# VikParuchuri/surya

Measured on AMD Instinct MI355X. Metric: text-lines/sec recognised (whole node), higher is better.
Workload: dtype bf16; 1 GPU; RecognitionPredictor device loop, 256 ragged 64x{128..512} crops/GPU, batch 256, max_tokens=48, REC-FULL synthetic weights (conditioned recipe, seed 0), tiles resident in HBM; parallelism=1 GPU, weights=conditioned

## Files before the change

surya_amd/csrc/common.h:

```cpp
#pragma once
#include <hip/hip_runtime.h>
#include <cstdlib>
#include <stdint.h>
#include <stdio.h>
#include <type_traits>

#include "../../include/surya_amd.h"

namespace sa {

typedef unsigned short bf16_t;
typedef __attribute__((ext_vector_type(4))) float f32x4;
typedef __attribute__((ext_vector_type(16))) float f32x16;
typedef __attribute__((ext_vector_type(8))) __bf16 bf16x8;
typedef unsigned int u32x4 __attribute__((ext_vector_type(4)));


#define SA_HIP(expr)                                                                                   \
    do {                                                                                               \
        hipError_t _e = (expr);                                                                        \
        if (_e != hipSuccess) {                                                                        \
            fprintf(stderr, "[surya_amd] %s:%d %s -> %s\n", __FILE__, __LINE__, #expr, hipGetErrorString(_e)); \
            return (int)_e;                                                                            \
        }                                                                                              \
// ... 228 lines not shown
    int graph = 0;
    int split_target = 256;
    int split_min_kt = 4;
    int split_max = 8;
    int bigtile = 3;
    int bigtile_any = 0;
    int big_m_split = -1;
    int big_m_gateup = -1;
    int mx_big_m_split = -1;
    int mx_big_m_gateup = -1;
    int gateup_ring = 2;
    int dring = 1;
    int dring_min_kt = 0;
    int conv_persist = 3;
    int dwconv_pipe = 2;
    int conv_lean = 1;
    int bigtile_ratio_pct = 0;
    int bigtile_min_k = 0;
    int glds = 2;
    int dattn = 4;
    int rnorm = 2;
    int ghead = 2;
    int fuse_embed = 1;
    int kvprefetch = 0;
    int lmhead = 1;
    int dattn_db = 0;
    int lay_ln = 1;
    int det_head_blk = 1;
    int det_fuse = 1023;
    int det_up4 = 1;
    int fmb_chunk = 64;
    int persist = 1;
    int ocrerr_cls_only = 1;
};
inline Tuning& tuning() { static Tuning t; return t; }
inline int& tuning_epoch() { static int e = 0; return e; }

inline void poison_arena(void* p, size_t bytes) {
    static const bool on = [] { const char* e = getenv("SURYA_AMD_POISON"); return e && e[0] == '1'; }();
    if (on) { (void)hipMemset(p, 0xFF, bytes); (void)hipDeviceSynchronize(); }
}

struct AttrOnce {
    size_t granted[64] = {};
    template <typename F> void ensure(F kern, size_t lds) {
        int dev = 0;
        (void)hipGetDevice(&dev);
        size_t& g = granted[dev & 63];
        if (lds > g || g == 0) {
            (void)hipFuncSetAttribute(reinterpret_cast<const void*>(kern), hipFuncAttributeMaxDynamicSharedMemorySize, (int)lds);
            g = lds > g ? lds : g;
            if (g == 0) g = 1;
        }
    }
};

constexpr int SA_ALT_NONE = 0x7fffffff;
__device__ __forceinline__ bool alt_after(float v, int c, float pv, int pc) { return (v < pv) | ((v == pv) & (c > pc)); }
__device__ __forceinline__ bool alt_before(float v, int c, float bv, int bc) { return (v > bv) | ((v == bv) & (c < bc)); }
__device__ __forceinline__ float2 alt_next(const float2* cand, int n, float pv, int pc) {
    float cb = -INFINITY;
    int ci = SA_ALT_NONE;
    for (int k = 0; k < n; ++k) {
        const float v = cand[k].x;
        const int cc = __float_as_int(cand[k].y);
        const bool take = (v > -INFINITY) & alt_after(v, cc, pv, pc) & alt_before(v, cc, cb, ci);
// ... 11 lines not shown
```

surya_amd/csrc/gemm.h:

```cpp
#pragma once
#include <algorithm>
#include <cstdlib>
#include <type_traits>

#include "common.h"
#include "fastdiv.h"

namespace sa {

enum GemmEpi { EPI_BIAS = 0, EPI_RESIDUAL = 1, EPI_GELU = 2, EPI_SWIGLU = 3, EPI_HARDSWISH = 4, EPI_RELU = 5, EPI_ARGMAX = 6, EPI_ROPE = 7,
               EPI_GEGLU = 8 ,
               EPI_ARGMAX_MASK = 9 ,
               EPI_TOPK = 10 ,
               EPI_FORCED = 11  };
constexpr bool epi_is_argmax(int epi) { return epi == EPI_ARGMAX || epi == EPI_ARGMAX_MASK || epi == EPI_TOPK || epi == EPI_FORCED; }
constexpr bool epi_is_masked(int epi) { return epi == EPI_ARGMAX_MASK || epi == EPI_TOPK; }

struct TokenMask {
    const uint32_t* table = nullptr;
    const int* slot_mask = nullptr;
    const int* row_slot = nullptr;
    int words = 0;
    __device__ __forceinline__ int id_of(int m, int M) const {
        const int gm = min(m, M - 1);
// ... 1578 lines not shown
    const bool prof = pf.enabled && pf.n < GemmProfiler::POOL;
    if (prof) (void)hipEventRecord(pf.ev[2 * pf.n], s);
    hipLaunchKernelGGL(kern, dim3(grid), dim3(512), lds, s, aa);
    if (prof) {
        (void)hipEventRecord(pf.ev[2 * pf.n + 1], s);
        pf.cfg_of[pf.n] = CONV ? 3 : gemm_cfg_id(BM, BN);
        pf.flops_of[pf.n] = CONV ? 2.0 * a.M * a.N * a.cTaps * a.cCin : 2.0 * a.M * a.N * a.K;
        const double outn = (EPI == EPI_SWIGLU || EPI == EPI_GEGLU) ? a.N / 2 : a.N;
        const double xelems = CONV ? (double)a.M / std::max(1, a.cHo * a.cWo) * a.cH * a.cW * a.cCin : (double)a.M * a.K;
        pf.bytes_of[pf.n] = (xelems + (double)a.N * a.K) * sizeof(TI) + (double)a.M * outn * sizeof(TO) +
                            (EPI == EPI_RESIDUAL ? (double)a.M * a.N * sizeof(TO) : 0.0);
        pf.slab_of[pf.n] = 0.0;
        ++pf.n;
    }
    return (int)hipGetLastError();
}

}
#include "gemm_ring.h"
namespace sa {

static inline bool gemm_misaligned(const void* p, size_t bytes) { return (reinterpret_cast<uintptr_t>(p) & (bytes - 1)) != 0; }
template <typename TI, typename TO>
static inline bool gemm_operands_ok(const GemmArgs<TI, TO>& a, bool with_r) {
    constexpr long CI = 16 / (long)sizeof(TI), CO = 16 / (long)sizeof(TO);
    if (a.K <= 0 || a.ldx % CI != 0 || a.ldw % CI != 0 || a.ldc % CO != 0) return false;
    if (gemm_misaligned(a.X, 16) || gemm_misaligned(a.W, 16) || gemm_misaligned(a.C, 16) || gemm_misaligned(a.part, 16)) return false;
    if (gemm_misaligned(a.bias, 4 * sizeof(TI))) return false;
    if (with_r && (a.ldr % CO != 0 || gemm_misaligned(a.R, 16))) return false;
    return true;
}

template <typename TI, typename TO, int EPI>
static inline int launch_gemm(const GemmArgs<TI, TO>& a, hipStream_t s) {
    if (a.M <= 0 || a.N <= 0) return SA_OK;
    if (!gemm_operands_ok(a, EPI == EPI_RESIDUAL)) return SA_ERR_SHAPE;
    if constexpr (EPI == EPI_ROPE) {
        if (!a.rope || gemm_misaligned(a.rope, 16) || a.rope_D <= 0 || a.rope_D % 4 != 0 || a.rope_cols < 4 || a.rope_cols % 4 != 0) return SA_ERR_SHAPE;
    }
    {
        const int n_out = (EPI == EPI_SWIGLU || EPI == EPI_GEGLU) ? a.N / 2 : a.N;
        if (a.K % Ty<TI>::KE != 0 || a.N % 4 != 0 || n_out % (16 / (int)sizeof(TO)) != 0 || a.ldc % (16 / (int)sizeof(TO)) != 0)
            return SA_ERR_SHAPE;
    }
    if constexpr (EPI == EPI_ARGMAX_MASK) {
        if (!a.tmask.table || !a.tmask.slot_mask || a.tmask.words != cdiv(a.N, 32)) return SA_ERR_ARG;
    }
    if constexpr (EPI == EPI_TOPK) {
        if (!a.alt || (a.tmask.table && (!a.tmask.slot_mask || a.tmask.words != cdiv(a.N, 32)))) return SA_ERR_ARG;
    }
    if constexpr (EPI == EPI_FORCED) {
        if (!a.forced.table || !a.forced.flogit || a.forced.stride <= 0) return SA_ERR_ARG;
    }
    if (a.M <= 256) {
        if constexpr (epi_is_argmax(EPI)) {
            if (a.N >= 64 * 512 && tuning().lmhead && (a.K / Ty<TI>::KE) % 2 == 0 && a.N % 4 == 0) {
                if constexpr (sizeof(TI) == 2)
                    if (tuning().lmhead == 2) return launch_gemm_cfg<TI, TO, 256, 320, 4, 2, EPI, false, 2, false, 2>(a, s);
                return launch_gemm_cfg<TI, TO, 256, 320, 4, 2, EPI, false, 2>(a, s);
            }
            if (a.N >= 64 * 512) return launch_gemm_cfg<TI, TO, 128, 128, 2, 2, EPI, false, 2>(a, s);
            return launch_gemm_cfg<TI, TO, 64, 64, 2, 2, EPI, false, 2>(a, s);
        }
        if (a.M > 128) {
            if (a.N >= 64 * 512) return launch_gemm_cfg<TI, TO, 128, 128, 2, 2, EPI, false, 2>(a, s);
            if constexpr (EPI == EPI_SWIGLU && sizeof(TI) == 2 && sizeof(TO) == 2) {
                const int rc = launch_gateup_ring(a, s);
// ... 17 lines not shown
            GemmArgs<TI, TO> g = a;
            g.mgroup = 1;
            int rc;
            if constexpr (sizeof(TI) == 2) {
                if (tuning().lmhead == 2) { rc = launch_gemm_cfg<TI, TO, 256, 320, 4, 2, EPI, false, 2, false, 2>(g, s); a.bn_used = g.bn_used; return rc; }
            }
            rc = launch_gemm_cfg<TI, TO, 256, 320, 4, 2, EPI, false, 2>(g, s);
            a.bn_used = g.bn_used;
            return rc;
        }
    }
    if constexpr (EPI == EPI_SWIGLU && sizeof(TI) == 2 && sizeof(TO) == 2) {
        const int mode = tuning().big_m_gateup;
        const int rb = cdiv(a.M, 256), t256 = rb * cdiv(a.N, 256);
        const int pick = mode >= 0 ? mode : ((rb >= 4 && t256 >= 160 && t256 < 256) ? 2 : 0);
        if (pick && (a.K / Ty<TI>::KE) % 2 == 0 && a.K / Ty<TI>::KE >= 4 && a.N % 8 == 0) {
            if (pick == 1) return launch_gemm_persist<TI, TO, EPI>(a, s);
            return launch_gemm_cfg<TI, TO, 256, 256, 4, 2, EPI, false, 8>(a, s);
        }
    }
    if (a.N <= 64 && a.M >= 128 * 256) return launch_gemm_cfg<TI, TO, 128, 64, 4, 1, EPI>(a, s);
    const long big = (long)cdiv(a.M, 128) * cdiv(a.N, 128);
    const int glds = tuning().glds;
    if constexpr (sizeof(TO) == 2) {
        const int bigtile = tuning().bigtile;
        const long t256 = (long)cdiv(a.M, 256) * cdiv(a.N, 256);
        const double ratio256 = tuning().bigtile_ratio_pct > 0 ? tuning().bigtile_ratio_pct / 100.0
                                                                : ((bigtile == 3 && sizeof(TI) == 2) ? 1.4 : 1.17);
        const double cost256 = (double)cdivl(t256, 256) * 256 * 4 / ratio256, cost128 = (double)cdivl(big, 512) * 512;
        if (bigtile && a.K >= tuning().bigtile_min_k && ((t256 >= 256 && cost256 <= cost128) || tuning().bigtile_any)) {
            if constexpr (!epi_is_argmax(EPI)) {
                const int nk = a.K / Ty<TI>::KE;
                if constexpr (sizeof(TI) == 2)
                    if (tuning().persist && nk >= 4 && nk % 2 == 0 && a.N % 8 == 0) return launch_gemm_persist<TI, TO, EPI>(a, s);
            }
            if constexpr (sizeof(TI) == 2 && !epi_is_argmax(EPI)) {
                if (bigtile == 2 && (a.K / Ty<TI>::KE) % 2 == 0) return launch_gemm_cfg<TI, TO, 256, 256, 2, 2, EPI, false, 2>(a, s);
                if (bigtile == 3 && (a.K / Ty<TI>::KE) % 2 == 0) return launch_gemm_cfg<TI, TO, 256, 256, 4, 2, EPI, false, 8>(a, s);
            }
            return launch_gemm_cfg<TI, TO, 256, 256, 4, 2, EPI, false, 2>(a, s);
        }
    }
    if (big >= 256) {
        if (glds == 2) return launch_gemm_cfg<TI, TO, 128, 128, 2, 2, EPI, false, 2>(a, s);
        if (glds == 3) return launch_gemm_cfg<TI, TO, 128, 128, 2, 2, EPI, false, 3>(a, s);
        return launch_gemm_cfg<TI, TO, 128, 128, 2, 2, EPI>(a, s);
    }
    return launch_gemm_cfg<TI, TO, 64, 64, 2, 2, EPI>(a, s);
}

static inline int pick_splitk(int tiles_n, int nk) {
    const Tuning& t = tuning();
    const int tiles = tiles_n * 4;
    int s = (t.split_target + tiles / 2) / tiles;
    s = std::min(s, nk / std::max(1, t.split_min_kt));
    return std::max(1, std::min(s, std::min(t.split_max, 8)));
}

template <typename TI>
static inline int launch_gemm_splitk(GemmArgs<TI, TI>& a, hipStream_t s) {
    if (a.M <= 0 || a.N <= 0) return SA_OK;
    if (a.K % Ty<TI>::KE != 0 || a.N % 4 != 0 || !a.part) return SA_ERR_SHAPE;
    if (!gemm_operands_ok(a, false)) return SA_ERR_SHAPE;
    const int nk = a.K / Ty<TI>::KE;
    a.splitk = pick_splitk(cdiv(a.N, 64), nk);
    if constexpr (sizeof(TI) == 2) {
        const int mode = tuning().big_m_split;
// ... 14 lines not shown
```

surya_amd/csrc/kernels.h:

```cpp
#pragma once
#include "common.h"

#ifndef SA_DBG_VARIANT
#define SA_DBG_VARIANT 0
#endif

namespace sa {

template <typename T>
__global__ void convert_tiles_kernel(const float* __restrict__ in, T* __restrict__ out, const int* __restrict__ src_row,
                                     int P, int kin, int kout) {
    const int row = blockIdx.x;
    const float* src = in + (long)src_row[row] * kin;
    T* dst = out + (long)row * kout;
    for (int c = threadIdx.x * 4; c < kout; c += blockDim.x * 4) {
        float v[4];
#pragma unroll
        for (int r = 0; r < 4; ++r) v[r] = (c + r < kin) ? src[c + r] : 0.f;
        store4(dst + c, v[0], v[1], v[2], v[3]);
    }
}

template <typename T>
__global__ __launch_bounds__(256) void rmsnorm_kernel(const T* __restrict__ x, long ldx, const T* __restrict__ w,
// ... 118 lines not shown
#pragma unroll
            for (int jj = 0; jj < 16; ++jj) {
                const int j = jb + jj;
                if (j < nk) {
                    const float pj = __expf(s[jj] - mnew);
                    lrun += pj;
                    const T* vr = vs + j * D + sl * DS;
#pragma unroll
                    for (int i = 0; i < DS; i += 4) {
                        float t4[4];
                        load4(vr + i, t4);
                        acc[i] += pj * t4[0]; acc[i + 1] += pj * t4[1]; acc[i + 2] += pj * t4[2]; acc[i + 3] += pj * t4[3];
                    }
                }
            }
        }
        __syncthreads();
    }
    if (valid) {
        const float inv = 1.0f / lrun;
        T* op = out + sg.o_off[seg] + (long)qi * o_row + (long)head * o_head + sl * DS;
#pragma unroll
        for (int i = 0; i < DS; i += 4) store4(op + i, acc[i] * inv, acc[i + 1] * inv, acc[i + 2] * inv, acc[i + 3] * inv);
    }
}

template <typename T>
__global__ void scatter_rows_kernel(const T* __restrict__ src, const int* __restrict__ dst_row, T* __restrict__ dst, int H) {
    const int r = blockIdx.x;
    const T* s = src + (long)r * H;
    T* d = dst + (long)dst_row[r] * H;
    for (int c = threadIdx.x * Ty<T>::V16; c < H; c += blockDim.x * Ty<T>::V16)
        *reinterpret_cast<uint4*>(d + c) = *reinterpret_cast<const uint4*>(s + c);
}

template <typename T>
__global__ void scatter_image_kernel(const T* __restrict__ merged, const T* __restrict__ hemb, const T* __restrict__ wemb,
                                     const int* __restrict__ dst_row, const int* __restrict__ hidx, const int* __restrict__ widx,
                                     T* __restrict__ embeds, int H) {
    const int r = blockIdx.x;
    const T* src = merged + (long)r * H;
    const T* he = hemb + (long)hidx[r] * H;
    const T* we = wemb + (long)widx[r] * H;
    T* dst = embeds + (long)dst_row[r] * H;
    for (int c = threadIdx.x * 4; c < H; c += blockDim.x * 4) {
        float a[4], b[4], d[4];
        load4(src + c, a); load4(he + c, b); load4(we + c, d);
        store4(dst + c, a[0] + Ty<T>::rnd(b[0] + d[0]), a[1] + Ty<T>::rnd(b[1] + d[1]), a[2] + Ty<T>::rnd(b[2] + d[2]),
               a[3] + Ty<T>::rnd(b[3] + d[3]));
    }
}

template <typename T>
__global__ void embed_tokens_kernel(const T* __restrict__ table, const int* __restrict__ ids, T* __restrict__ x, int H) {
    const int t = blockIdx.x;
    const int id = ids[t];
    if (id < 0) return;
    const uint4* src = reinterpret_cast<const uint4*>(table + (long)id * H);
    uint4* dst = reinterpret_cast<uint4*>(x + (long)t * H);
    for (int c = threadIdx.x; c < H / Ty<T>::V16; c += blockDim.x) dst[c] = src[c];
}

template <typename T>
__global__ void rope_table_kernel(const float* __restrict__ inv_freq, float2* __restrict__ table, int Tmax, int half) {
    const int idx = blockIdx.x * blockDim.x + threadIdx.x;
    if (idx >= Tmax * half) return;
// ... 512 lines not shown
    hipLaunchKernelGGL(rmsnorm_kernel<T>, dim3(cdiv(rows, 4)), dim3(256), 0, s, x, ldx, w, y, ldy, src_row, rows, C, eps);
    return (int)hipGetLastError();
}

template <typename T>
int launch_convert_tiles(const float* in, T* out, const int* src_row, int P, int kin, int kout, hipStream_t s) {
    if (P <= 0) return SA_OK;
    if (kout % 4 || kin > kout) return SA_ERR_SHAPE;
    hipLaunchKernelGGL(convert_tiles_kernel<T>, dim3(P), dim3(64), 0, s, in, out, src_row, P, kin, kout);
    return (int)hipGetLastError();
}
inline int launch_rope_vision_table(const int* pos_hw, const float* inv_freq, float2* tab, int P, int D, hipStream_t s) {
    if (P <= 0) return SA_OK;
    if (D <= 0 || D % 4) return SA_ERR_SHAPE;
    hipLaunchKernelGGL(rope_vision_table_kernel, dim3((unsigned)cdivl((long)P * (D / 2), 256)), dim3(256), 0, s, pos_hw, inv_freq, tab, P, D);
    return (int)hipGetLastError();
}
template <typename T>
int launch_scatter_image(const T* merged, const T* hemb, const T* wemb, const int* dst_row, const int* hidx, const int* widx, T* embeds, int rows,
                         int H, hipStream_t s) {
    if (rows <= 0) return SA_OK;
    if (H % 4) return SA_ERR_SHAPE;
    hipLaunchKernelGGL(scatter_image_kernel<T>, dim3(rows), dim3(128), 0, s, merged, hemb, wemb, dst_row, hidx, widx, embeds, H);
    return (int)hipGetLastError();
}
template <typename T>
int launch_scatter_rows(const T* src, const int* dst_row, T* dst, int rows, int H, hipStream_t s) {
    if (rows <= 0) return SA_OK;
    if (H % Ty<T>::V16) return SA_ERR_SHAPE;
    hipLaunchKernelGGL(scatter_rows_kernel<T>, dim3((unsigned)rows), dim3(128), 0, s, src, dst_row, dst, H);
    return (int)hipGetLastError();
}
template <typename T>
int launch_embed_tokens(const T* table, const int* ids, T* x, int rows, int H, hipStream_t s) {
    if (rows <= 0) return SA_OK;
    if (H % Ty<T>::V16) return SA_ERR_SHAPE;
    hipLaunchKernelGGL(embed_tokens_kernel<T>, dim3(rows), dim3(128), 0, s, table, ids, x, H);
    return (int)hipGetLastError();
}
template <typename T>
int launch_rope_table(const float* inv_freq, float2* table, int Tmax, int half, hipStream_t s) {
    if (Tmax <= 0 || half <= 0 || (long)Tmax * half > 0x7fffffffL) return SA_ERR_SHAPE;
    hipLaunchKernelGGL(rope_table_kernel<T>, dim3(cdiv(Tmax * half, 256)), dim3(256), 0, s, inv_freq, table, Tmax, half);
    return (int)hipGetLastError();
}
template <typename T>
int launch_rope_kv_append(T* qkv, const int* tok_slot, const int* tok_pos, const float2* rope_cs, T* kc, T* vc, int M, int nq, int nkv, int D,
                          int Tmax, hipStream_t s) {
    if (M <= 0) return SA_OK;
    if (D <= 0 || D % 2 || nq <= 0 || nkv <= 0) return SA_ERR_SHAPE;
    hipLaunchKernelGGL(rope_kv_append_kernel<T>, dim3(M), dim3(256), 0, s, qkv, tok_slot, tok_pos, rope_cs, kc, vc, nq, nkv, D, Tmax);
    return (int)hipGetLastError();
}

template <typename T>
int launch_reduce_norm(const float* part, int S, int M, T* x, const T* w, T* y, int H, float eps, uint8_t* y8, uint8_t* sy, int srows,
                       const KvPrefetch& pf, hipStream_t s) {
    const int threads = cdiv(H / 4, 64) * 64;
    if (threads > 1024 || H % 4) return SA_ERR_UNSUPPORTED;
    const int grid = pf.base ? 2 * M : M;
#define SA_RNORM(SL) hipLaunchKernelGGL((splitk_residual_norm_kernel<T, SL>), dim3(grid), dim3(threads), 0, s, part, S, M, x, (const T*)nullptr, \
                                        w, y, H, eps, y8, sy, srows, pf)
    if (tuning().rnorm == 1 || S > 4) SA_RNORM(8);
    else if (S > 2) SA_RNORM(4);
    else SA_RNORM(2);
#undef SA_RNORM
// ... 52 lines not shown
```

surya_amd/csrc/rec_engine.h:

```cpp
#pragma once
#include <memory>

#include "rec_state.h"
#include "decode_attn.h"
#include "kv_fanout.h"
#include "kv_store.h"
#include "attn_mfma.h"
#include "beam.h"

namespace sa {

struct EncPlan {
    int P = 0;
    std::vector<int> src_row, pos_hw, merged_src, hidx, widx;
    std::vector<int> win_cu, img_cu;
};

static int plan_encoder(const surya_rec_config& c, const int32_t* grid_hw, int n, EncPlan& pl) {
    const int mg = c.merge, unit = mg * mg, vw = c.window_tokens;
    pl = EncPlan();
    pl.win_cu.push_back(0);
    pl.img_cu.push_back(0);
    int tok_base = 0;
    for (int im = 0; im < n; ++im) {
// ... 21 lines not shown
                        ++cnt;
                    }
                if (cnt) pl.win_cu.push_back(pl.win_cu.back() + cnt * unit);
            }
        tok_base += lh * lw;
        pl.img_cu.push_back(pl.img_cu.back() + h * w);
    }
    pl.P = pl.img_cu.back();
    return SA_OK;
}

struct SegLists {
    std::vector<int> tile_seg, tile_q0, seg_len;
    std::vector<long> q_off, k_off, v_off, o_off;
    void add_tiles(int seg, int L) {
        for (int q0 = 0; q0 < L; q0 += 64) { tile_seg.push_back(seg); tile_q0.push_back(q0); }
    }
};

static AttnSegs stage_segs(Stager& st, const SegLists& s) {
    AttnSegs a;
    a.tile_seg = st.put(s.tile_seg); a.tile_q0 = st.put(s.tile_q0); a.seg_len = st.put(s.seg_len);
    a.q_off = st.put(s.q_off); a.k_off = st.put(s.k_off); a.v_off = st.put(s.v_off); a.o_off = st.put(s.o_off);
    return a;
}

template <int I> using HeadEpi = std::integral_constant<int, I>;

template <typename T>
struct RecModel : RecBase {
    T* emb_ahead = nullptr;
    T *tiles_t, *ex, *eh, *eqkv, *emlp, *emh, *emerged;
    T *dx, *dh, *dqkv, *dattn, *dmlp, *dlast;
    float* logits;
    float2* erope;
    float4* amax;
    float2* rope_cs;
    float* part;
    T *kcache, *vcache;
    static constexpr bool MX_OK = std::is_same<T, bf16_t>::value;
    const T* W(int idx) const { return reinterpret_cast<const T*>(w[idx]); }
    const T* WE(int l, int k) const { return W(SA_RW_ENC(l, k)); }
    const T* WD(int l, int k) const { return W(SA_RW_DEC(c.enc_depth, l, k)); }

    static size_t layout(const surya_rec_config& c, RecModel* m) {
        Carve cv;
        const size_t Pm = c.max_patches, Tm = std::max(c.max_prefill_tokens, c.max_slots), S = c.max_slots;
        const int unit = c.merge * c.merge;
        const size_t qkv_d = (size_t)(c.dec_heads + 2 * c.dec_kv_heads) * c.dec_head_dim;
        size_t o_tiles = cv.take(Pm * c.patch_dim_pad * sizeof(T));
        size_t o_ex = cv.take(Pm * c.enc_hidden * sizeof(T));
        size_t o_eh = cv.take(Pm * c.enc_hidden * sizeof(T));
        size_t o_eqkv = cv.take(Pm * 3 * c.enc_hidden * sizeof(T));
        size_t o_emlp = cv.take(Pm * c.enc_inter_pad * sizeof(T));
        size_t o_emh = cv.take(Pm * c.enc_hidden * sizeof(T));
        size_t o_erope = cv.take(Pm * (size_t)(c.enc_hidden / c.enc_heads / 2) * sizeof(float2));
        size_t o_emerged = cv.take(Pm / unit * c.enc_out_hidden * sizeof(T));
        size_t o_dx = cv.take(Tm * c.dec_hidden * sizeof(T));
        size_t o_dh = cv.take(Tm * c.dec_hidden * sizeof(T));
        size_t o_dqkv = cv.take(Tm * qkv_d * sizeof(T));
        size_t o_dattn = cv.take(Tm * c.dec_heads * c.dec_head_dim * sizeof(T));
        size_t o_dmlp = cv.take(Tm * c.dec_inter * sizeof(T));
        size_t o_dlast = cv.take(S * c.dec_hidden * sizeof(T));
        size_t o_ahead = cv.take(Tm * c.dec_hidden * sizeof(T));
        size_t o_logits = cv.take(S * (size_t)c.vocab * sizeof(float));
        size_t o_amax = cv.take(S * (size_t)cdiv(c.vocab, 32) * sizeof(float4));
        size_t o_rope = cv.take((size_t)c.max_kv_len * (c.dec_head_dim / 2) * sizeof(float2));
        size_t o_part = cv.take((size_t)8 * S * std::max(qkv_d, (size_t)c.dec_hidden) * sizeof(float));
        const size_t kv_elems = (size_t)c.dec_layers * S * c.dec_kv_heads * c.max_kv_len * c.dec_head_dim;
        size_t o_k = cv.take(kv_elems * sizeof(T));
        size_t o_v = cv.take(kv_elems * sizeof(T));
        size_t o_kvlen = cv.take(S * sizeof(int));
        size_t o_next = cv.take(S * sizeof(int));
        size_t o_active = cv.take(S * sizeof(int));
        size_t o_rowlen = cv.take(S * sizeof(int));
        size_t o_out = cv.take((size_t)SA_MAX_STEPS * S * 8 * sizeof(int));
        if (m) {
            char* b = m->blk[RecBase::B_MAIN].dev;
            m->tiles_t = (T*)(b + o_tiles); m->ex = (T*)(b + o_ex); m->eh = (T*)(b + o_eh); m->eqkv = (T*)(b + o_eqkv);
            m->emlp = (T*)(b + o_emlp); m->emh = (T*)(b + o_emh); m->emerged = (T*)(b + o_emerged); m->erope = (float2*)(b + o_erope);
            m->dx = (T*)(b + o_dx); m->dh = (T*)(b + o_dh); m->dqkv = (T*)(b + o_dqkv); m->dattn = (T*)(b + o_dattn);
            m->dmlp = (T*)(b + o_dmlp); m->dlast = (T*)(b + o_dlast); m->emb_ahead = (T*)(b + o_ahead); m->logits = (float*)(b + o_logits); m->amax = (float4*)(b + o_amax);
            m->part = (float*)(b + o_part); m->rope_cs = (float2*)(b + o_rope);
            m->kcache = (T*)(b + o_k); m->vcache = (T*)(b + o_v);
            m->kv_len = (int*)(b + o_kvlen); m->next_token = (int*)(b + o_next); m->active_dev = (int*)(b + o_active); m->row_len = (int*)(b + o_rowlen);
            m->out_token = (int*)(b + o_out);
            m->out_score = (float*)(m->out_token + (size_t)SA_MAX_STEPS * S);
            m->out_bbox = (int*)(m->out_score + (size_t)SA_MAX_STEPS * S);
            m->out_bytes = (size_t)SA_MAX_STEPS * S * 8 * sizeof(int);
        }
        return cv.off;
    }

    int init(const surya_rec_config& cfg, const void* const* weights, int n) {
        c = cfg;
        w.assign(weights, weights + n);
        arena_bytes = layout(c, nullptr);
        for (auto& o : outs) o.slots = c.max_slots;
        const size_t mirror = (size_t)SA_MAX_STEPS * c.max_slots * 32;
        int rc = blk[B_MAIN].alloc(arena_bytes, mirror, 0, {}, false);
        if (rc) return rc;
        poison_arena(blk[B_MAIN].dev, arena_bytes);
        layout(c, this);
        if ((rc = launch_rope_table<T>(reinterpret_cast<const float*>(w[SA_RW_DEC_INVFREQ]), rope_cs, c.max_kv_len, c.dec_head_dim / 2, 0))) return rc;
        SA_HIP(hipMemset(kv_len, 0, c.max_slots * sizeof(int)));
        SA_HIP(hipMemset(next_token, 0, c.max_slots * sizeof(int)));
        SA_HIP(hipMemset(out_token, 0, out_bytes));
        StepOutputs& base = outs[STEPS_BASE];
        base.add(out_token, 4); base.add(out_score, 4); base.add(out_bbox, 24);
        base.mirrored[0] = base.mirrored[1] = true;
        base.host = blk[B_MAIN].host;
        if (base.host_bytes() != mirror) return SA_ERR_STATE;
        const size_t Pm = c.max_patches, Tm = std::max(c.max_prefill_tokens, c.max_slots);
        rc = st.init((Pm * 8 + Tm * 8 + (size_t)c.max_slots * 64) * sizeof(int) + (1 << 20));
// ... 119 lines not shown
    int encode_only(const float* tiles, const int32_t* grid_hw, int n, void* out, hipStream_t s) override {
        if (c.enc_out_hidden != c.dec_hidden) return SA_ERR_SHAPE;
        long ntok = 0;
        for (int i = 0; i < n; ++i) ntok += (long)grid_hw[2 * i] * grid_hw[2 * i + 1] / (c.merge * c.merge);
        std::vector<int> ident(ntok);
        for (long i = 0; i < ntok; ++i) ident[i] = (int)i;
        return encode(tiles, grid_hw, n, ident, reinterpret_cast<T*>(out), s);
    }

    int encode_ahead(const float* tiles, const int32_t* grid_hw, int n, hipStream_t s) override {
        if (c.enc_out_hidden != c.dec_hidden) return SA_ERR_SHAPE;
        if (n == 0) {
            ahead_consumed = ahead_tokens = 0;
            return SA_OK;
        }
        if (n < 0 || !tiles || !grid_hw) return SA_ERR_ARG;
        if (ahead_consumed != ahead_tokens) return SA_ERR_STATE;
        long ntok = 0;
        for (int i = 0; i < n; ++i) ntok += (long)grid_hw[2 * i] * grid_hw[2 * i + 1] / (c.merge * c.merge);
        if (ntok > std::max(c.max_prefill_tokens, c.max_slots)) return SA_ERR_SHAPE;
        std::vector<int> ident(ntok);
        for (long i = 0; i < ntok; ++i) ident[i] = (int)i;
        SA_HIP(hipEventRecord(ev_ahead_in, s));
        SA_HIP(hipStreamWaitEvent(estream, ev_ahead_in, 0));
        if (ahead_free_recorded) SA_HIP(hipStreamWaitEvent(estream, ev_ahead_free, 0));
        int rc = encode(tiles, grid_hw, n, ident, emb_ahead, estream, st_enc);
        if (rc) return rc;
        SA_HIP(hipEventRecord(ev_ahead_done, estream));
        ahead_tokens = ntok;
        ahead_consumed = 0;
        return SA_OK;
    }

    int decoder_layers_prefill(int M, const int* d_tok_slot, const int* d_tok_pos, const AttnSegs* sg, int n_tiles, hipStream_t s) {
        const int Hd = c.dec_hidden, nq = c.dec_heads, nkv = c.dec_kv_heads, d = c.dec_head_dim, I = c.dec_inter;
        const int qkv_d = (nq + 2 * nkv) * d;
        const float scale = 1.0f / sqrtf((float)d);
        const size_t layer_kv = (size_t)c.max_slots * nkv * c.max_kv_len * d;
        const float* inv_freq = reinterpret_cast<const float*>(w[SA_RW_DEC_INVFREQ]);
        int rc;
        for (int l = 0; l < c.dec_layers; ++l) {
            T* kc = kcache + l * layer_kv;
            T* vc = vcache + l * layer_kv;
            if ((rc = rmsnorm(dx, Hd, WD(l, SA_RD_LN1), dh, Hd, nullptr, M, Hd, c.dec_eps, s))) return rc;
            if ((rc = gemm<EPI_BIAS>(dh, Hd, WD(l, SA_RD_QKV_W), Hd, dqkv, qkv_d, WD(l, SA_RD_QKV_B), nullptr, 0, M, qkv_d, Hd, s)))
                return rc;
            if ((rc = launch_rope_kv_append<T>(dqkv, d_tok_slot, d_tok_pos, rope_cs, kc, vc, M, nq, nkv, d, c.max_kv_len, s))) return rc;
            if constexpr (std::is_same<T, bf16_t>::value) {
                if (kv8) {
                    const size_t l8 = (size_t)c.max_slots * nkv, T8 = tmax8();
                    if ((rc = launch_kv8_quant_rows(d, kc, vc, d_tok_slot, d_tok_pos, M, k8c + l * l8 * c.max_kv_len * d, v8tc + l * l8 * d * T8,
                                                    ksc8 + l * l8 * T8, vsc8 + l * l8 * T8, nkv, c.max_kv_len, s))) return rc;
                }
            }
            if ((rc = launch_attn<T>(d, dqkv, kc, vc, dattn, *sg, n_tiles, nq, qkv_d, d, d, (long)c.max_kv_len * d, (long)nq * d, d,
                                     nq / nkv, 1, scale, s))) return rc;
            if ((rc = gemm<EPI_RESIDUAL>(dattn, (long)nq * d, WD(l, SA_RD_O_W), (long)nq * d, dx, Hd, nullptr, dx, Hd, M, Hd, nq * d,
                                         s))) return rc;
            if ((rc = rmsnorm(dx, Hd, WD(l, SA_RD_LN2), dh, Hd, nullptr, M, Hd, c.dec_eps, s))) return rc;
            if ((rc = gemm<EPI_SWIGLU>(dh, Hd, WD(l, SA_RD_GU_W), Hd, dmlp, I, nullptr, nullptr, 0, M, 2 * I, Hd, s))) return rc;
            if ((rc = gemm<EPI_RESIDUAL>(dmlp, I, WD(l, SA_RD_DOWN_W), I, dx, Hd, nullptr, dx, Hd, M, Hd, I, s))) return rc;
        }
        return SA_OK;
    }

    struct Half { int r0, M; float* part; hipStream_t s; };

    int splitk_gemm(const T* X, long ldx, const T* Wt, long ldw, int M, int N, int K, float* part_, int* S, hipStream_t s) {
        GemmArgs<T, T> a{X, ldx, Wt, ldw, nullptr, 0, nullptr, nullptr, 0, M, N, K, 1, part_};
        int rc = launch_gemm_splitk<T>(a, s);
        *S = a.splitk;
        return rc;
    }
    int reduce_residual_norm(int S, int M, const float* part_, T* x, const T* wnorm, T* y, hipStream_t s, uint8_t* y8 = nullptr,
                             uint8_t* sy = nullptr, const T* pf_cache = nullptr, const Half* h = nullptr) {
        KvPrefetch pf;
        if (pf_cache && h && tuning().kvprefetch && (c.dec_head_dim * sizeof(T)) % 16 == 0) {
            pf.base = reinterpret_cast<const unsigned char*>(pf_cache);
            pf.slots = active_dev + h->r0; pf.lens = row_len + h->r0;
            pf.head_stride = (long)c.max_kv_len * c.dec_head_dim * sizeof(T);
            pf.slot_stride = pf.head_stride * c.dec_kv_heads;
            pf.heads = c.dec_kv_heads; pf.row_bytes = c.dec_head_dim * (int)sizeof(T); pf.max_rows = c.max_kv_len;
        }
        return launch_reduce_norm<T>(part_, S, M, x, wnorm, y, c.dec_hidden, c.dec_eps, y8, sy, c.max_slots, pf, s);
    }

    int set_kv_fp8(int on) override {
        if constexpr (!std::is_same<T, bf16_t>::value) return on ? SA_ERR_UNSUPPORTED : SA_OK;
        if (on && excluded(M_KV8)) return SA_ERR_STATE;
// ... 324 lines not shown
        const int* d_last = st_small.put(last_row);
        const int* d_keep = keep_first ? st_small.put(keep_first, n_seqs) : nullptr;
        if (!d_last || (keep_first && !d_keep)) return SA_ERR_NOMEM;
        if ((rc = st_small.flush(s))) return rc;
        {
            st.begin();
            const int* d_ids = st.put(ids);
            if (!d_ids) return SA_ERR_NOMEM;
            if ((rc = st.flush(s))) return rc;
            if ((rc = launch_embed_tokens<T>(W(SA_RW_TOK_EMBED), d_ids, dx, Ttot, c.dec_hidden, s))) return rc;
        }
        if (n_images > 0 && tiles) {
            if ((rc = encode(tiles, grid_hw, n_images, img_pos, dx, s))) return rc;
        } else if (n_images > 0) {
            if (ahead_consumed + ntok > ahead_tokens) return SA_ERR_STATE;
            st.begin();
            const int* d_img = st.put(img_pos);
            if (!d_img) return SA_ERR_NOMEM;
            if ((rc = st.flush(s))) return rc;
            SA_HIP(hipStreamWaitEvent(s, ev_ahead_done, 0));
            if ((rc = launch_scatter_rows<T>(emb_ahead + ahead_consumed * c.dec_hidden, d_img, dx, (int)ntok, c.dec_hidden, s))) return rc;
            ahead_consumed += ntok;
            SA_HIP(hipEventRecord(ev_ahead_free, s));
            ahead_free_recorded = true;
        }
        st.begin();
        const int* d_tok_slot = st.put(tok_slot);
        const int* d_tok_pos = st.put(tok_pos);
        AttnSegs d_sg = stage_segs(st, sg);
        if (!d_sg.o_off) return SA_ERR_NOMEM;
        if (!fan_offsets) {
            if ((rc = st.flush(s))) return rc;
            hipLaunchKernelGGL(set_slot_state_kernel, dim3(cdiv(n_seqs, 256)), dim3(256), 0, s, d_slots, d_lens, kv_len, n_seqs);
            if ((rc = decoder_layers_prefill(Ttot, d_tok_slot, d_tok_pos, &d_sg, (int)sg.tile_seg.size(), s))) return rc;
            if (keep_first && (rc = launch_kv_keep<T>(kcache, vcache, store_k, store_v, d_slots, d_keep, d_lens, n_seqs, c.dec_layers, c.max_slots,
                                                      c.dec_kv_heads, c.max_kv_len, c.dec_head_dim, store_cap, dx, d_last, store_h, c.dec_hidden,
                                                      Ttot, s))) return rc;
            if ((rc = heads(n_seqs, d_last, d_slots, 0, 0, false, s)) || beam == 0) return rc;
            return beam_step(d_slots, 1, n_seqs, 0, 1, s);
        }
        const int F = fan_offsets[n_seqs], n_dst = (int)f_dst.size();
        const int* d_fslots = st.put(fan_slots, F);
        const int* d_flens = st.put(f_lens);
        const int* d_flast = st.put(f_last);
        const int* d_foff = st.put(f_off);
        if (f_dst.empty()) f_dst.push_back(-1);
        const int* d_fdst = st.put(f_dst);
        if (!d_fslots || !d_flens || !d_flast || !d_foff || !d_fdst) return SA_ERR_NOMEM;
        if ((rc = st.flush(s))) return rc;
        hipLaunchKernelGGL(set_slot_state_kernel, dim3(cdiv(F, 256)), dim3(256), 0, s, d_fslots, d_flens, kv_len, F);
        if ((rc = decoder_layers_prefill(Ttot, d_tok_slot, d_tok_pos, &d_sg, (int)sg.tile_seg.size(), s))) return rc;
        if ((rc = launch_kv_fanout<T>(kcache, vcache, d_slots, d_foff, d_fdst, d_lens, n_seqs, n_dst, c.dec_layers, c.max_slots, c.dec_kv_heads,
                                      c.max_kv_len, c.dec_head_dim, s))) return rc;
        return heads(F, d_flast, d_fslots, 0, 0, false, s);
    }

    int decode_eager(int M, int n_steps, int step0, hipStream_t s) {
        int rc;
        const Half h{0, M, part, s};
        const bool fuse = can_fuse_embed() && beam == 0;
        if (h_len.size() < (size_t)c.max_slots) h_len.resize(c.max_slots, 0);
        for (int step = 0; step < n_steps; ++step) {
            ctx_bound = 0;
            for (int a : h_active) {
                ctx_bound = std::max(ctx_bound, h_len[a] + 1);
                h_len[a] = std::min(h_len[a] + 1, c.max_kv_len);
            }
            if ((step == 0 || !fuse) && (rc = decode_embed(h))) return rc;
            for (int l = 0; l < c.dec_layers; ++l)
                if ((rc = decode_layer(l, h))) return rc;
            if ((rc = heads(M, nullptr, active_dev, step0 + step, 1, true, s, fuse && step + 1 < n_steps))) return rc;
            if (beam > 0 && (rc = beam_step(active_dev, beam, M / beam, step0 + step, 0, s))) return rc;
        }
        return SA_OK;
    }

    int decode(int n_steps, hipStream_t s) override { return decode_steps(n_steps, 0, s); }

    int decode_async(int n_steps, int ring, hipStream_t s) override {
        if (n_steps < 0 || n_steps > SA_MAX_STEPS / 2 || ring < 0 || ring > 1) return SA_ERR_ARG;
        const int rc = decode_steps(n_steps, StepOutputs::ring_step(ring), s);
        return rc ? rc : mirror_steps(n_steps, ring, s);
    }

// ... 69 lines not shown
```

surya_amd/csrc/rec_model.hip:

```cpp
#include "rec_engine.h"
#include "rec_ops.h"
#include "rec_prep.h"
#include "rec_rectify.h"
#include "rec_adjust.h"

namespace sa {

template <int D, int MAXG>
static int decode_attn_flash(const DecodeAttnArgs<bf16_t>& a, hipStream_t s) {
    const Tuning& t = tuning();
    if (t.dattn == 3) return decode_attn_as<decode_attn_flash_kernel<D, MAXG>>(a, decode_attn_flash_lds<D, MAXG>(), s, a.out8, a.sout, a.srows);
    if (t.dattn_db == 1 || (t.dattn_db == 0 && !t.graph && a.ctx_bound > 128 && a.rows * a.nkv <= 256))
        return decode_attn_as<decode_attn_flash2_kernel<D, MAXG, true>>(a, decode_attn_flash2_lds<D, MAXG, true>(), s, a.out8, a.sout, a.srows);
    return decode_attn_as<decode_attn_flash2_kernel<D, MAXG, false>>(a, decode_attn_flash2_lds<D, MAXG, false>(), s, a.out8, a.sout, a.srows);
}
template <typename T>
int launch_decode_attn(const DecodeAttnArgs<T>& a, hipStream_t s) {
    const int G = a.nq / a.nkv, d = a.d;
    if constexpr (std::is_same<T, bf16_t>::value) {
        if (d == 128 && G <= 5) return decode_attn_flash<128, 5>(a, s);
        if (d == 128 && G <= 8) return decode_attn_flash<128, 8>(a, s);
        if (d == 64 && G <= 8) return decode_attn_flash<64, 8>(a, s);
        if (d == 32 && G <= 8) return decode_attn_flash<32, 8>(a, s);
    }
// ... 619 lines not shown

int surya_rec_preprocess(const uint8_t* pages, const void* lines, int n_lines, uint8_t* mask_arena, float* mid_arena, float* tiles,
                         int patch_size, int merge_size, float pad_value, const float* mean, const float* std, int any_poly,
                         int max_stage1_width, int pixel_stride, void* stream) {
    if (!pages || !lines || !tiles || !mean || !std || n_lines < 0 || patch_size <= 0 || merge_size <= 0) return SA_ERR_ARG;
    if (pixel_stride != 3 && pixel_stride != 4) return SA_ERR_ARG;
    sa::prep::PrepArgs p;
    p.pages = pages; p.lines = reinterpret_cast<const sa::prep::LineDesc*>(lines); p.n_lines = n_lines;
    p.mask = mask_arena; p.mid = mid_arena; p.tiles = tiles; p.ps = patch_size; p.merge = merge_size; p.pad = pad_value;
    for (int i = 0; i < 3; ++i) { p.mean[i] = mean[i]; p.std[i] = std[i]; }
    p.max_mid_w = max_stage1_width;
    p.pix = pixel_stride;
    return sa::prep::prep_run(p, any_poly, max_stage1_width > 0, (hipStream_t)stream);
}

int surya_rec_rectify(const uint8_t* pages, const void* descs, int n, uint8_t* out, int pixel_stride, int max_w, int max_h, void* stream) {
    return sa::prep::rectify_run(pages, reinterpret_cast<const sa::prep::RectifyDesc*>(descs), n, out, pixel_stride, max_w, max_h,
                                 (hipStream_t)stream);
}

int surya_rec_adjust_contrast(const uint8_t* pages, const void* descs, int n, uint8_t* out, uint8_t* mask_arena, void* work, int32_t* lo_hi,
                              int pixel_stride, void* stream) {
    return sa::prep::adjust_run(pages, reinterpret_cast<const sa::adjust::AdjustDesc*>(descs), n, out, mask_arena, work, lo_hi, pixel_stride,
                                (hipStream_t)stream);
}

int surya_set_tuning(const char* key, int value) {
    if (!key) return SA_ERR_ARG;
    Tuning& t = tuning();
    struct { const char* k; int* v; } tab[] = {
        {"graph", &t.graph}, {"split_target", &t.split_target}, {"split_min_kt", &t.split_min_kt}, {"split_max", &t.split_max},
        {"bigtile", &t.bigtile}, {"bigtile_any", &t.bigtile_any}, {"conv_lean", &t.conv_lean}, {"conv_persist", &t.conv_persist}, {"dwconv_pipe", &t.dwconv_pipe}, {"bigtile_ratio_pct", &t.bigtile_ratio_pct}, {"gateup_ring", &t.gateup_ring}, {"dring", &t.dring}, {"dring_min_kt", &t.dring_min_kt}, {"big_m_split", &t.big_m_split}, {"big_m_gateup", &t.big_m_gateup}, {"mx_big_m_split", &t.mx_big_m_split}, {"mx_big_m_gateup", &t.mx_big_m_gateup}, {"glds", &t.glds}, {"bigtile_min_k", &t.bigtile_min_k}, {"dattn", &t.dattn}, {"rnorm", &t.rnorm},
        {"ghead", &t.ghead}, {"fuse_embed", &t.fuse_embed}, {"persist", &t.persist}, {"lmhead", &t.lmhead}, {"kvprefetch", &t.kvprefetch},
        {"dattn_db", &t.dattn_db}, {"lay_ln", &t.lay_ln}, {"det_head_blk", &t.det_head_blk}, {"det_fuse", &t.det_fuse}, {"det_up4", &t.det_up4}, {"fmb_chunk", &t.fmb_chunk}, {"ocrerr_cls_only", &t.ocrerr_cls_only}};
    for (auto& e : tab)
        if (!strcmp(e.k, key)) {
            if (*e.v != value) ++tuning_epoch();
            *e.v = value;
            return SA_OK;
        }
    return SA_ERR_ARG;
}

int surya_gemm_ring_status(int reset) {
    const int a = sa::ring_error(reset != 0), b = sa::rec_f16_ring_error(reset != 0);
    return a ? a : b;
}

int surya_prof_enable(int on) {
    GemmProfiler& pf = gemm_profiler();
    if (on) pf.start(); else pf.enabled = false;
    return SA_OK;
}

__global__ void prof_null_kernel() {}

int surya_prof_event_overhead(void* stream, double* ms) {
    if (!ms) return SA_ERR_ARG;
    hipStream_t s = (hipStream_t)stream;
    constexpr int N = 201;
    hipEvent_t ev[2 * N];
    for (auto& e : ev) SA_HIP(hipEventCreate(&e));
    for (int i = 0; i < 32; ++i) hipLaunchKernelGGL(prof_null_kernel, dim3(1), dim3(64), 0, s);
    for (int i = 0; i < N; ++i) {
        SA_HIP(hipEventRecord(ev[2 * i], s));
        hipLaunchKernelGGL(prof_null_kernel, dim3(1), dim3(64), 0, s);
        SA_HIP(hipEventRecord(ev[2 * i + 1], s));
// ... 149 lines not shown
```

Measured before the change: 3174 lines/s.

## Split large GEMMs by rows for wave quantization and trim last prefill layer

Adds a row-split path in the big-tile GEMM dispatcher. When a cost model predicts it is cheaper, it runs whole waves of 256x256 persistent tiles on the leading rows and dispatches the remainder rows separately, to reduce wave-quantization tail waste. This is enabled by default. It also adds an optional (default off) prefill trim that computes the last decoder layer's O-proj and MLP only for each sequence's last token, via new gather/scatter kernels and scratch buffers. The split adds an extra launch, and the heuristic cost constants may misjudge some shapes.

New measurement: 3207 lines/s (median of 6 runs). 1.0% higher.

```diff
diff --git a/surya_amd/csrc/common.h b/surya_amd/csrc/common.h
--- a/surya_amd/csrc/common.h
+++ b/surya_amd/csrc/common.h
@@ -284,6 +284,8 @@
     int fmb_chunk = 64;
     int persist = 1;
     int ocrerr_cls_only = 1;
+    int gemm_rowsplit = 1;
+    int prefill_trim = 0;
 };
 inline Tuning& tuning() { static Tuning t; return t; }
 inline int& tuning_epoch() { static int e = 0; return e; }
diff --git a/surya_amd/csrc/gemm.h b/surya_amd/csrc/gemm.h
--- a/surya_amd/csrc/gemm.h
+++ b/surya_amd/csrc/gemm.h
@@ -1634,7 +1634,7 @@
 }
 
 template <typename TI, typename TO, int EPI>
-static inline int launch_gemm(const GemmArgs<TI, TO>& a, hipStream_t s) {
+static inline int launch_gemm(const GemmArgs<TI, TO>& a, hipStream_t s, bool rowsplit = true) {
     if (a.M <= 0 || a.N <= 0) return SA_OK;
     if (!gemm_operands_ok(a, EPI == EPI_RESIDUAL)) return SA_ERR_SHAPE;
     if constexpr (EPI == EPI_ROPE) {
@@ -1718,7 +1718,34 @@
             if constexpr (!epi_is_argmax(EPI)) {
                 const int nk = a.K / Ty<TI>::KE;
                 if constexpr (sizeof(TI) == 2)
-                    if (tuning().persist && nk >= 4 && nk % 2 == 0 && a.N % 8 == 0) return launch_gemm_persist<TI, TO, EPI>(a, s);
+                    if (tuning().persist && nk >= 4 && nk % 2 == 0 && a.N % 8 == 0) {
+                        const int mode = rowsplit ? tuning().gemm_rowsplit : 0;
+                        const int tn = cdiv(a.N, 256);
+                        const long whole = t256 / 256;
+                        const int tm1 = (int)(whole * 256 / tn);
+                        const int M1 = tm1 * 256, M2 = a.M - M1;
+                        if (mode > 0 && whole > 0 && tm1 > 0 && M2 > 0) {
+                            const long big2 = (long)cdiv(M2, 128) * cdiv(a.N, 128), t2 = (long)cdiv(M2, 256) * tn, last = big2 % 512;
+                            const double c256r = (double)cdivl(t2, 256) * 256 * 4 / ratio256, c128r = (double)cdivl(big2, 512) * 512;
+                            const double r128 = 1.2 * 512, part = 0.72 * r128 * std::max(0.3, (double)last / 256);
+                            const double rem = ((t2 >= 256 && c256r <= c128r) || tuning().bigtile_any)
+                                                   ? c256r : (double)(big2 / 512) * r128 + (last == 0 ? 0.0 : (last <= 256 ? part : r128));
+                            const double cost_split = (double)whole * 256 * 4 / ratio256 + rem + 163840.0 / a.K;
+                            if (mode == 2 || (cost_split < 0.97 * cost256 && cost_split < cost128)) {
+                                GemmArgs<TI, TO> p = a, q = a;
+                                p.M = M1;
+                                q.M = M2;
+                                q.X = a.X + (long)M1 * a.ldx;
+                                q.C = a.C + (long)M1 * a.ldc;
+                                if (a.R) q.R = a.R + (long)M1 * a.ldr;
+                                if constexpr (EPI == EPI_ROPE) q.rope = a.rope + (long)M1 * (a.rope_D / 2);
+                                const int rc = launch_gemm_persist<TI, TO, EPI>(p, s);
+                                if (rc) return rc;
+                                return launch_gemm<TI, TO, EPI>(q, s, false);
+                            }
+                        }
+                        return launch_gemm_persist<TI, TO, EPI>(a, s);
+                    }
             }
             if constexpr (sizeof(TI) == 2 && !epi_is_argmax(EPI)) {
                 if (bigtile == 2 && (a.K / Ty<TI>::KE) % 2 == 0) return launch_gemm_cfg<TI, TO, 256, 256, 2, 2, EPI, false, 2>(a, s);
diff --git a/surya_amd/csrc/kernels.h b/surya_amd/csrc/kernels.h
--- a/surya_amd/csrc/kernels.h
+++ b/surya_amd/csrc/kernels.h
@@ -174,6 +174,17 @@
     T* d = dst + (long)dst_row[r] * H;
     for (int c = threadIdx.x * Ty<T>::V16; c < H; c += blockDim.x * Ty<T>::V16)
         *reinterpret_cast<uint4*>(d + c) = *reinterpret_cast<const uint4*>(s + c);
+}
+
+template <typename T>
+__global__ void gather_rows2_kernel(const T* __restrict__ a, int Ha, const T* __restrict__ b, int Hb, const int* __restrict__ row,
+                                    T* __restrict__ da, T* __restrict__ db) {
+    const int r = blockIdx.x;
+    const long src = row[r];
+    for (int c = threadIdx.x * Ty<T>::V16; c < Ha; c += blockDim.x * Ty<T>::V16)
+        *reinterpret_cast<uint4*>(da + (long)r * Ha + c) = *reinterpret_cast<const uint4*>(a + src * Ha + c);
+    for (int c = threadIdx.x * Ty<T>::V16; c < Hb; c += blockDim.x * Ty<T>::V16)
+        *reinterpret_cast<uint4*>(db + (long)r * Hb + c) = *reinterpret_cast<const uint4*>(b + src * Hb + c);
 }
 
 template <typename T>
@@ -752,6 +763,13 @@
     return (int)hipGetLastError();
 }
 template <typename T>
+int launch_gather_rows2(const T* a, int Ha, const T* b, int Hb, const int* row, T* da, T* db, int rows, hipStream_t s) {
+    if (rows <= 0) return SA_OK;
+    if (Ha % Ty<T>::V16 || Hb % Ty<T>::V16) return SA_ERR_SHAPE;
+    hipLaunchKernelGGL(gather_rows2_kernel<T>, dim3((unsigned)rows), dim3(128), 0, s, a, Ha, b, Hb, row, da, db);
+    return (int)hipGetLastError();
+}
+template <typename T>
 int launch_embed_tokens(const T* table, const int* ids, T* x, int rows, int H, hipStream_t s) {
     if (rows <= 0) return SA_OK;
     if (H % Ty<T>::V16) return SA_ERR_SHAPE;
diff --git a/surya_amd/csrc/rec_engine.h b/surya_amd/csrc/rec_engine.h
--- a/surya_amd/csrc/rec_engine.h
+++ b/surya_amd/csrc/rec_engine.h
@@ -77,6 +77,7 @@
     T* emb_ahead = nullptr;
     T *tiles_t, *ex, *eh, *eqkv, *emlp, *emh, *emerged;
     T *dx, *dh, *dqkv, *dattn, *dmlp, *dlast;
+    T *tx, *th, *tattn, *tmlp;
     float* logits;
     float2* erope;
     float4* amax;
@@ -107,6 +108,10 @@
         size_t o_dattn = cv.take(Tm * c.dec_heads * c.dec_head_dim * sizeof(T));
         size_t o_dmlp = cv.take(Tm * c.dec_inter * sizeof(T));
         size_t o_dlast = cv.take(S * c.dec_hidden * sizeof(T));
+        size_t o_tx = cv.take(S * c.dec_hidden * sizeof(T));
+        size_t o_th = cv.take(S * c.dec_hidden * sizeof(T));
+        size_t o_tattn = cv.take(S * c.dec_heads * c.dec_head_dim * sizeof(T));
+        size_t o_tmlp = cv.take(S * c.dec_inter * sizeof(T));
         size_t o_ahead = cv.take(Tm * c.dec_hidden * sizeof(T));
         size_t o_logits = cv.take(S * (size_t)c.vocab * sizeof(float));
         size_t o_amax = cv.take(S * (size_t)cdiv(c.vocab, 32) * sizeof(float4));
@@ -125,6 +130,7 @@
             m->tiles_t = (T*)(b + o_tiles); m->ex = (T*)(b + o_ex); m->eh = (T*)(b + o_eh); m->eqkv = (T*)(b + o_eqkv);
             m->emlp = (T*)(b + o_emlp); m->emh = (T*)(b + o_emh); m->emerged = (T*)(b + o_emerged); m->erope = (float2*)(b + o_erope);
             m->dx = (T*)(b + o_dx); m->dh = (T*)(b + o_dh); m->dqkv = (T*)(b + o_dqkv); m->dattn = (T*)(b + o_dattn);
+            m->tx = (T*)(b + o_tx); m->th = (T*)(b + o_th); m->tattn = (T*)(b + o_tattn); m->tmlp = (T*)(b + o_tmlp);
             m->dmlp = (T*)(b + o_dmlp); m->dlast = (T*)(b + o_dlast); m->emb_ahead = (T*)(b + o_ahead); m->logits = (float*)(b + o_logits); m->amax = (float4*)(b + o_amax);
             m->part = (float*)(b + o_part); m->rope_cs = (float2*)(b + o_rope);
             m->kcache = (T*)(b + o_k); m->vcache = (T*)(b + o_v);
@@ -310,7 +316,8 @@
         return SA_OK;
     }
 
-    int decoder_layers_prefill(int M, const int* d_tok_slot, const int* d_tok_pos, const AttnSegs* sg, int n_tiles, hipStream_t s) {
+    int decoder_layers_prefill(int M, const int* d_tok_slot, const int* d_tok_pos, const AttnSegs* sg, int n_tiles, const int* d_last, int n_seqs,
+                               hipStream_t s) {
         const int Hd = c.dec_hidden, nq = c.dec_heads, nkv = c.dec_kv_heads, d = c.dec_head_dim, I = c.dec_inter;
         const int qkv_d = (nq + 2 * nkv) * d;
         const float scale = 1.0f / sqrtf((float)d);
@@ -333,6 +340,15 @@
             }
             if ((rc = launch_attn<T>(d, dqkv, kc, vc, dattn, *sg, n_tiles, nq, qkv_d, d, d, (long)c.max_kv_len * d, (long)nq * d, d,
                                      nq / nkv, 1, scale, s))) return rc;
+            if (l + 1 == c.dec_layers && tuning().prefill_trim && d_last && n_seqs > 0 && n_seqs <= c.max_slots && M >= 4 * n_seqs) {
+                const int A = nq * d, R = n_seqs;
+                if ((rc = launch_gather_rows2<T>(dattn, A, dx, Hd, d_last, tattn, tx, R, s))) return rc;
+                if ((rc = gemm<EPI_RESIDUAL>(tattn, A, WD(l, SA_RD_O_W), A, tx, Hd, nullptr, tx, Hd, R, Hd, A, s))) return rc;
+                if ((rc = rmsnorm(tx, Hd, WD(l, SA_RD_LN2), th, Hd, nullptr, R, Hd, c.dec_eps, s))) return rc;
+                if ((rc = gemm<EPI_SWIGLU>(th, Hd, WD(l, SA_RD_GU_W), Hd, tmlp, I, nullptr, nullptr, 0, R, 2 * I, Hd, s))) return rc;
+                if ((rc = gemm<EPI_RESIDUAL>(tmlp, I, WD(l, SA_RD_DOWN_W), I, tx, Hd, nullptr, tx, Hd, R, Hd, I, s))) return rc;
+                return launch_scatter_rows<T>(tx, d_last, dx, R, Hd, s);
+            }
             if ((rc = gemm<EPI_RESIDUAL>(dattn, (long)nq * d, WD(l, SA_RD_O_W), (long)nq * d, dx, Hd, nullptr, dx, Hd, M, Hd, nq * d,
                                          s))) return rc;
             if ((rc = rmsnorm(dx, Hd, WD(l, SA_RD_LN2), dh, Hd, nullptr, M, Hd, c.dec_eps, s))) return rc;
@@ -723,7 +739,7 @@
         if (!fan_offsets) {
             if ((rc = st.flush(s))) return rc;
             hipLaunchKernelGGL(set_slot_state_kernel, dim3(cdiv(n_seqs, 256)), dim3(256), 0, s, d_slots, d_lens, kv_len, n_seqs);
-            if ((rc = decoder_layers_prefill(Ttot, d_tok_slot, d_tok_pos, &d_sg, (int)sg.tile_seg.size(), s))) return rc;
+            if ((rc = decoder_layers_prefill(Ttot, d_tok_slot, d_tok_pos, &d_sg, (int)sg.tile_seg.size(), d_last, n_seqs, s))) return rc;
             if (keep_first && (rc = launch_kv_keep<T>(kcache, vcache, store_k, store_v, d_slots, d_keep, d_lens, n_seqs, c.dec_layers, c.max_slots,
                                                       c.dec_kv_heads, c.max_kv_len, c.dec_head_dim, store_cap, dx, d_last, store_h, c.dec_hidden,
                                                       Ttot, s))) return rc;
@@ -740,7 +756,7 @@
         if (!d_fslots || !d_flens || !d_flast || !d_foff || !d_fdst) return SA_ERR_NOMEM;
         if ((rc = st.flush(s))) return rc;
         hipLaunchKernelGGL(set_slot_state_kernel, dim3(cdiv(F, 256)), dim3(256), 0, s, d_fslots, d_flens, kv_len, F);
-        if ((rc = decoder_layers_prefill(Ttot, d_tok_slot, d_tok_pos, &d_sg, (int)sg.tile_seg.size(), s))) return rc;
+        if ((rc = decoder_layers_prefill(Ttot, d_tok_slot, d_tok_pos, &d_sg, (int)sg.tile_seg.size(), d_last, n_seqs, s))) return rc;
         if ((rc = launch_kv_fanout<T>(kcache, vcache, d_slots, d_foff, d_fdst, d_lens, n_seqs, n_dst, c.dec_layers, c.max_slots, c.dec_kv_heads,
                                       c.max_kv_len, c.dec_head_dim, s))) return rc;
         return heads(F, d_flast, d_fslots, 0, 0, false, s);
diff --git a/surya_amd/csrc/rec_model.hip b/surya_amd/csrc/rec_model.hip
--- a/surya_amd/csrc/rec_model.hip
+++ b/surya_amd/csrc/rec_model.hip
@@ -675,7 +675,8 @@
         {"graph", &t.graph}, {"split_target", &t.split_target}, {"split_min_kt", &t.split_min_kt}, {"split_max", &t.split_max},
         {"bigtile", &t.bigtile}, {"bigtile_any", &t.bigtile_any}, {"conv_lean", &t.conv_lean}, {"conv_persist", &t.conv_persist}, {"dwconv_pipe", &t.dwconv_pipe}, {"bigtile_ratio_pct", &t.bigtile_ratio_pct}, {"gateup_ring", &t.gateup_ring}, {"dring", &t.dring}, {"dring_min_kt", &t.dring_min_kt}, {"big_m_split", &t.big_m_split}, {"big_m_gateup", &t.big_m_gateup}, {"mx_big_m_split", &t.mx_big_m_split}, {"mx_big_m_gateup", &t.mx_big_m_gateup}, {"glds", &t.glds}, {"bigtile_min_k", &t.bigtile_min_k}, {"dattn", &t.dattn}, {"rnorm", &t.rnorm},
         {"ghead", &t.ghead}, {"fuse_embed", &t.fuse_embed}, {"persist", &t.persist}, {"lmhead", &t.lmhead}, {"kvprefetch", &t.kvprefetch},
-        {"dattn_db", &t.dattn_db}, {"lay_ln", &t.lay_ln}, {"det_head_blk", &t.det_head_blk}, {"det_fuse", &t.det_fuse}, {"det_up4", &t.det_up4}, {"fmb_chunk", &t.fmb_chunk}, {"ocrerr_cls_only", &t.ocrerr_cls_only}};
+        {"dattn_db", &t.dattn_db}, {"lay_ln", &t.lay_ln}, {"det_head_blk", &t.det_head_blk}, {"det_fuse", &t.det_fuse}, {"det_up4", &t.det_up4}, {"fmb_chunk", &t.fmb_chunk}, {"ocrerr_cls_only", &t.ocrerr_cls_only},
+        {"gemm_rowsplit", &t.gemm_rowsplit}, {"prefill_trim", &t.prefill_trim}};
     for (auto& e : tab)
         if (!strcmp(e.k, key)) {
             if (*e.v != value) ++tuning_epoch();
```
